# kocurvik/mdrp

Hardware: NVIDIA B200
Metric: image_pairs_per_sec (higher is better)
Workload: dtype f64

## Files before the change

mdrp_b200/csrc/repose_b200.cu:

```cuda
#include <cuda.h>
#include <cuda_runtime.h>
#include <algorithm>
#include <cstdio>
#include <cstdlib>
#include <cstring>
#include <string>
#include <type_traits>
#include <vector>

#include "rp_kernels.cuh"

using namespace rp;

namespace {

std::string g_create_error;

struct DevBuf {
    void *p = nullptr;
    size_t cap = 0;
    cudaError_t reserve(size_t bytes) {
        if (bytes <= cap) return cudaSuccess;
        if (p) cudaFree(p);
        p = nullptr;
// ... 3 lines not shown
        if (e == cudaSuccess) cap = want;
        return e;
    }
    void release() {
        if (p) cudaFree(p);
        p = nullptr;
        cap = 0;
    }
    template <class T>
    T *as() const { return (T *)p; }
};

enum { B_OFFS, B_PAIRS, B_PTS64, B_PTS32, B_BEAR, B_SAMPLES, B_MODELS, B_HYPITER, B_SCORE, B_COUNT, B_SEGCNT,
       B_ITEMPFX, B_SCALARS, B_EVENTS, B_NEVENTS, B_LOMODELS, B_LOOFEV, B_LOCOUNT, B_PROBLIST, B_LOSCORE,
       B_LOCNT, B_LOITEMPFX, B_BEST, B_FINSTART, B_FINSCORE, B_FINCNT, B_ONES, B_ONEPFX, B_ENABLE, B_STATS,
       B_PTS32P, B_UB, B_LB, B_FIRSTCNT, B_FIRSTPFX, B_B0, B_S0, B_SURVLIST, B_SURVCNT, B_SURVPFX, B_WAVECUR, B_WAVECNT,
       B_MASK, B_IN_X1, B_IN_X2, B_IN_D1, B_IN_D2, B_IN_CAMS, B_TMP0, B_TMP1, B_TMP2,
       B_MASK_B, B_IN_X1_B, B_IN_X2_B, B_IN_D1_B, B_IN_D2_B, B_IN_CAMS_B, B_TMP0_B, B_TMP1_B,
       B_FEAT, B_TCOUT, B_TCLIST, B_TCLISTCNT, B_TCLISTPFX, B_PAIRCNT, B_TCPFX, B_TCSPLIT,
       B_PAIRFLAGS, B_SUB_IDX, B_SUB_SRC, B_SUB_DST, B_SUB_X1, B_SUB_X2, B_SUB_D1, B_SUB_D2, B_SUB_CAMS, B_SUB_MODELS,
       B_SUB_STATS, B_SUB_MASK,
       B_STG_X1, B_STG_X2, B_STG_D1, B_STG_D2, B_STG_X1_B, B_STG_X2_B, B_STG_D1_B, B_STG_D2_B,
       B_QUAL, B_QUAL_B, B_ORDOFFS, B_ORDOFFS_B, B_PERM, B_PERM_B, B_KSORT, B_KSORT_B, B_ORDSCR,
       B_GATHER_Q, B_NBUF };

struct Scalars {
    int n_items, n_lo_items, n_one_items, n_prob, n_pairs_scalar, any_flag, reserved0, n_first_items;
    int n_surv_items, bound_work, lm_work, score_work;
    unsigned long long point_scores, lm_iters, n_survivors, evaluated_ps;
    long long n_hyp;
    int n_tc_items, n_tcsel_items;
    unsigned long long tc_evaluated, tc_selected, lm_flops;
};

constexpr int N_EVENTS = 29;

}

struct rp_ctx {
    int device = 0;
    int sms = 148;
    std::string err;
    int64_t launches = 0;
    cudaStream_t stream = nullptr;
    cudaStream_t copy_stream = nullptr;
    DevBuf buf[B_NBUF];
    cudaEvent_t ev[N_EVENTS];
    double last_ms[16] = {0};
    double prev_h2d_ms = 0.0, prev_dev_ms = 0.0;
    int64_t last_cnt[16] = {0};
    size_t workspace_budget = (size_t)80 << 30;
    bool prune = true;
    int head = HB;
    bool waves = true;
    int lm_warp = 0xf;
    int head_small = 32;
    int mid_end = 256;
    int mid_ends[4] = {256, 0, 0, 0}, n_mid = 1;
    bool tc = true;
    int tc_two_pass = -115;
    void *encode_tiled = nullptr;
    int ev_cap0 = EV;
    std::vector<int32_t> pair_status;
    int occ_score[4] = {0}, occ_lm[4] = {0};
};

namespace {

#define CK(call)                                                                                     \
    do {                                                                                             \
        cudaError_t e_ = (call);                                                                     \
        if (e_ != cudaSuccess) {                                                                     \
            char b_[512];                                                                            \
            snprintf(b_, sizeof b_, "%s failed at %s:%d: %s", #call, __FILE__, __LINE__,             \
                     cudaGetErrorString(e_));                                                        \
            ctx->err = b_;                                                                           \
            return RP_ERR_CUDA;                                                                      \
        }                                                                                            \
// ... 55 lines not shown
    }
    LAUNCHED();
    return RP_OK;
}

int launch_bound(rp_ctx *ctx, bool pose, const BoundArgs &a, cudaStream_t st) {
    CK(cudaMemsetAsync(a.work_counter, 0, sizeof(int), st));
    if (pose) bound_kernel<true><<<occupancy_grid(ctx, bound_kernel<true>, SCORE_THREADS), SCORE_THREADS, 0, st>>>(a);
    else bound_kernel<false><<<occupancy_grid(ctx, bound_kernel<false>, SCORE_THREADS), SCORE_THREADS, 0, st>>>(a);
    LAUNCHED();
    return RP_OK;
}

int launch_lm(rp_ctx *ctx, int variant, const LMArgs &a, long long expected_problems, cudaStream_t st) {
    ctx->launches++;
    (void)expected_problems;
    LMArgs la = a;
    la.work_counter = &ctx->buf[B_SCALARS].as<Scalars>()->lm_work;
    la.warp_kernel = (ctx->lm_warp >> variant) & 1;
    la.warp_single = (ctx->lm_warp >> 4) & 1;
    CK(cudaMemsetAsync(la.work_counter, 0, sizeof(int), st));
    CK((cudaError_t)launch_lm_kernel(ctx->sms, variant, la, st));
    return RP_OK;
}

int launch_solve(rp_ctx *ctx, int variant, const SolveArgs &a, int n_pairs, cudaStream_t st) {
    dim3 grid(a.nseg, n_pairs);
    const bool generic = getenv("RP_SOLVE_GENERIC") != nullptr;
    switch (variant) {
    case RP_CALIB:
        if (generic) solve_kernel<RP_CALIB><<<grid, SOLVE_THREADS, 0, st>>>(a);
        else solve2_kernel<P3PCand><<<grid, SOLVE_THREADS, 0, st>>>(a);
        break;
    case RP_CALIB_SHIFT:
        if (generic) solve_kernel<RP_CALIB_SHIFT><<<grid, SOLVE_THREADS, 0, st>>>(a);
        else solve2_kernel<ShiftCand><<<grid, SOLVE_THREADS, 0, st>>>(a);
        break;
    case RP_SHARED:
        if (generic) solve_kernel<RP_SHARED><<<grid, SOLVE_THREADS, 0, st>>>(a);
        else solve2_kernel<FocalCand><<<grid, SOLVE_THREADS, 0, st>>>(a);
        break;
    default: solve_kernel<RP_VARYING><<<grid, SOLVE_THREADS, 0, st>>>(a); break;
    }
    LAUNCHED();
    return RP_OK;
}
// ... 77 lines not shown
    CK(B[B_PAIRFLAGS].reserve(sizeof(int) * P));
    CK(B[B_LOCNT].reserve(sizeof(int) * (size_t)P * ev_cap));
    CK(B[B_LOITEMPFX].reserve(sizeof(int) * (P + 1)));
    CK(B[B_BEST].reserve(sizeof(Model) * P));
    CK(B[B_FINSTART].reserve(sizeof(Model) * P));
    CK(B[B_FINSCORE].reserve(sizeof(double) * P));
    CK(B[B_FINCNT].reserve(sizeof(int) * P));
    CK(B[B_ONES].reserve(sizeof(int) * P));
    CK(B[B_ONEPFX].reserve(sizeof(int) * (P + 1)));
    CK(B[B_ENABLE].reserve(sizeof(int) * P));
    CK(B[B_STATS].reserve(sizeof(rp_stats) * P));
    if (ctx->prune) {
        CK(B[B_UB].reserve(sizeof(int) * slots));
        CK(B[B_LB].reserve(sizeof(float) * slots));
        CK(B[B_SURVLIST].reserve(sizeof(int) * slots));
        CK(B[B_FIRSTCNT].reserve(sizeof(int) * P));
        CK(B[B_FIRSTPFX].reserve(sizeof(int) * (P + 1)));
        CK(B[B_B0].reserve(sizeof(int) * P));
        CK(B[B_S0].reserve(sizeof(double) * P));
        CK(B[B_SURVCNT].reserve(sizeof(int) * P));
        CK(B[B_WAVECUR].reserve(sizeof(int) * P)); CK(B[B_WAVECNT].reserve(sizeof(int) * P));
        CK(B[B_SURVPFX].reserve(sizeof(int) * (P + 1)));
    }
    const bool use_tc = ctx->prune && ctx->tc;
    if (use_tc) {
        CK(B[B_FEAT].reserve(128 * (size_t)std::max<long long>(N, 1) + 128 * tc::NT));
        CK(B[B_TCOUT].reserve(sizeof(int) * slots));
        CK(B[B_TCLIST].reserve(sizeof(int) * slots));
        CK(B[B_TCLISTCNT].reserve(sizeof(int) * P));
        CK(B[B_TCLISTPFX].reserve(sizeof(int) * (P + 1)));
        CK(B[B_PAIRCNT].reserve(sizeof(int) * P));
        CK(B[B_TCSPLIT].reserve(sizeof(int) * P));
        CK(B[B_TCPFX].reserve(sizeof(int) * (P + 1)));
    }

    Scalars *sc = B[B_SCALARS].as<Scalars>();
    PairParams *pairs = B[B_PAIRS].as<PairParams>();
    Pt64 *pts64 = B[B_PTS64].as<Pt64>();
    float4 *pts32 = B[B_PTS32].as<float4>();
    Bear *bear = B[B_BEAR].as<Bear>();
    int *samples = B[B_SAMPLES].as<int>();
    Model *models = B[B_MODELS].as<Model>();
    int *hyp_iter = B[B_HYPITER].as<int>();
    double *score = B[B_SCORE].as<double>();
    int *count = B[B_COUNT].as<int>();
    int *seg_count = B[B_SEGCNT].as<int>();
// ... 185 lines not shown
    {
        ScanArgs a;
        a.n_pairs = P; a.nseg = nseg; a.seg_count = seg_count; a.score = score; a.count = count;
        a.events = B[B_EVENTS].as<int>(); a.n_events = B[B_NEVENTS].as<int>(); a.ev_cap = ev_cap;
        a.pair_flags = B[B_PAIRFLAGS].as<int>(); a.any_flag = &sc->any_flag;
        scan_kernel<<<cdiv((long long)P * 32, 256), 256, 0, st>>>(a);
        LAUNCHED();
        LoPrepArgs l;
        l.n_pairs = P; l.nseg = nseg; l.events = a.events; l.n_events = a.n_events; l.hyp_iter = hyp_iter; l.ev_cap = ev_cap;
        l.models = models; l.lo_models = B[B_LOMODELS].as<Model>(); l.lo_of_event = B[B_LOOFEV].as<int>();
        l.lo_count = B[B_LOCOUNT].as<int>(); l.prob_list = B[B_PROBLIST].as<int>(); l.n_prob = &sc->n_prob;
        lo_prepare_kernel<<<cdiv(P, 128), 128, 0, st>>>(l);
        LAUNCHED();
    }
    CK(cudaEventRecord(ev[5], st));
    LMArgs la;
    memset(&la, 0, sizeof la);
    la.pairs = pairs; la.pts64 = pts64; la.d1 = io.d1; la.d2 = io.d2;
    la.weight_sampson = opt.weight_sampson; la.gradient_tol = 1e-10; la.step_tol = 1e-8;
    la.initial_lambda = 1e-3; la.min_lambda = 1e-10; la.max_lambda = 1e10;
    la.loss_scale_override = -1.0; la.scale_reproj_override = -1.0;
    la.lm_iters = &sc->lm_iters;
    la.lm_flops = &sc->lm_flops;
    {
        la.prob_list = B[B_PROBLIST].as<int>(); la.n_prob = &sc->n_prob; la.prob_per_pair = ev_cap;
        la.models = B[B_LOMODELS].as<Model>(); la.use_final = 0;
        int rc = launch_lm(ctx, variant, la, (long long)P * 8, st);
        if (rc) return rc;
    }
    CK(cudaEventRecord(ev[6], st));
    {
        build_items_kernel<<<1, 1024, 0, st>>>(P, B[B_LOCOUNT].as<int>(), B[B_LOITEMPFX].as<int>(), &sc->n_lo_items, nullptr);
        LAUNCHED();
        ScoreArgs s2 = sa;
        s2.slot_list = nullptr; s2.list_stride = 0;
        s2.n_groups = P; s2.grp_stride = ev_cap; s2.grp_per_pair = 1; s2.grp_cnt = B[B_LOCOUNT].as<int>();
        s2.item_prefix = B[B_LOITEMPFX].as<int>(); s2.n_items = &sc->n_lo_items; s2.models = B[B_LOMODELS].as<Model>();
        s2.score = B[B_LOSCORE].as<double>(); s2.count = B[B_LOCNT].as<int>(); s2.point_scores = nullptr;
        int rc = launch_score(ctx, pose, false, s2, st);
        if (rc) return rc;
        MergeArgs m;
        m.n_pairs = P; m.nseg = nseg; m.iters = iters; m.pairs = pairs; m.events = B[B_EVENTS].as<int>();
        m.min_iterations = opt.min_iterations; m.max_iterations = opt.max_iterations;
        m.dyn_num_trials_mult = opt.dyn_num_trials_mult; m.log_prob_missing = log(1.0 - opt.success_prob);
        m.hyp_iter = hyp_iter; m.ev_cap = ev_cap; m.pair_flags = B[B_PAIRFLAGS].as<int>(); m.any_flag = &sc->any_flag;
        m.n_events = B[B_NEVENTS].as<int>(); m.lo_of_event = B[B_LOOFEV].as<int>(); m.score = score; m.count = count;
// ... 143 lines not shown

int rerun_flagged(rp_ctx *ctx, int variant, const rp_options &opt, const ChunkIO &io, const std::vector<long long> &rel,
                  const std::vector<int> &flags0, int iters0, int64_t p0, cudaStream_t st) {
    DevBuf *B = ctx->buf;
    const bool pose = variant == RP_CALIB || variant == RP_CALIB_SHIFT;
    std::vector<int> todo;
    for (int i = 0; i < io.n_pairs; ++i)
        if (flags0[(size_t)i]) todo.push_back(i);
    int iters = iters0, ev_cap = ctx->ev_cap0;
    std::vector<int> flags_of((size_t)io.n_pairs, 0);
    for (int i : todo) flags_of[(size_t)i] = flags0[(size_t)i];
    while (!todo.empty()) {
        bool any_more = false, any_ovf = false;
        for (int i : todo) {
            any_more |= (flags_of[(size_t)i] & PAIR_FLAG_NEED_MORE) != 0;
            any_ovf |= (flags_of[(size_t)i] & PAIR_FLAG_OVERFLOW) != 0;
            ctx->pair_status[(size_t)(p0 + i)] |= ((flags_of[(size_t)i] & PAIR_FLAG_NEED_MORE) ? RP_PAIR_CONTINUED : 0) |
                                                  ((flags_of[(size_t)i] & PAIR_FLAG_OVERFLOW) ? RP_PAIR_EVENTS_RERUN : 0);
        }
        if (any_more) iters = (int)std::min<int64_t>(opt.max_iterations, (int64_t)iters * 4);
        const int slots_pp = std::max(1, cdiv(iters, SEG)) * 4 * SEG;
        if (any_ovf) ev_cap = (int)std::min<int64_t>((int64_t)ev_cap * 8, slots_pp);
        std::vector<int> next;
        size_t pos = 0;
        while (pos < todo.size()) {
            size_t end = pos;
            size_t bytes = 0;
            long long npts = 0;
            while (end < todo.size()) {
                const long long n = rel[(size_t)todo[end] + 1] - rel[(size_t)todo[end]];
                const size_t b = bytes_per_pair(iters, n, ev_cap);
                if (end > pos && bytes + b > ctx->workspace_budget) break;
                bytes += b;
                npts += n;
                ++end;
            }
            const int S = (int)(end - pos);
            std::vector<int> idx((size_t)S);
            std::vector<long long> src((size_t)S), dst((size_t)S + 1, 0);
            for (int j = 0; j < S; ++j) {
                idx[(size_t)j] = todo[pos + j];
                src[(size_t)j] = rel[(size_t)idx[(size_t)j]];
                dst[(size_t)j + 1] = dst[(size_t)j] + (rel[(size_t)idx[(size_t)j] + 1] - rel[(size_t)idx[(size_t)j]]);
            }
            const size_t nn = (size_t)std::max<long long>(npts, 1);
            int rc = RP_OK;
            std::vector<int> flags;
            do {
                cudaError_t e = cudaSuccess;
                (void)e;
// ... 56 lines not shown
                  cudaStream_t st) {
    constexpr bool f32 = std::is_same<In, float>::value;
    const bool ordered = quality != nullptr;
    const bool staged = f32 || ordered;
    int rc = check_common(ctx, variant, n_pairs, offsets, opt_in);
    if (rc) return rc;
    CK(cudaSetDevice(ctx->device));
    rp_options opt = *opt_in;
    if (variant == RP_CALIB && opt.estimate_shift) variant = RP_CALIB_SHIFT;
    if (variant == RP_CALIB_SHIFT) opt.estimate_shift = 1;
    const bool pose = variant == RP_CALIB || variant == RP_CALIB_SHIFT;
    if (pose && !cams && n_pairs > 0) return fail(ctx, RP_ERR_INVALID, "calibrated variants need cams");
    memset(ctx->last_ms, 0, sizeof ctx->last_ms);
    memset(ctx->last_cnt, 0, sizeof ctx->last_cnt);
    ctx->pair_status.assign((size_t)n_pairs, RP_PAIR_OK);
    if (n_pairs == 0) return RP_OK;
    const long long Ntot = offsets[n_pairs] - offsets[0];
    const int iters0 = opt.min_iterations < opt.max_iterations
                           ? (int)std::min<int64_t>(opt.max_iterations, opt.min_iterations + 1)
                           : (int)opt.max_iterations;
    size_t in_bytes = f32 ? 48 : 0;
    if (ordered) in_bytes = host_io ? 2 * (6 * sizeof(In) + 4 + 4 + 1) : 48 + 4 + 1;
    const size_t bpp = bytes_per_pair(iters0, Ntot / n_pairs + 1, ctx->ev_cap0, in_bytes);
    int64_t chunk = (int64_t)std::max<size_t>(1, ctx->workspace_budget / bpp);
    chunk = std::min<int64_t>(chunk, 32768);
    std::vector<long long> rel;
    DevBuf *B = ctx->buf;
    std::vector<int64_t> bounds(1, 0);
    {
        int64_t first = 0;
        if (host_io && n_pairs >= 1024 && !getenv("RP_NO_LEAD_CHUNK")) {
            double f = 0.125;
            if (ctx->prev_h2d_ms > 0.0 && ctx->prev_dev_ms > 0.0) f = ctx->prev_h2d_ms / (ctx->prev_h2d_ms + ctx->prev_dev_ms);
            f = std::min(1.0 / 3.0, std::max(1.0 / 32.0, f));
            first = std::min<int64_t>(std::min<int64_t>(n_pairs, chunk), std::max<int64_t>(256, (int64_t)(f * (double)n_pairs)));
        }
        if (first > 0) bounds.push_back(first);
        const int64_t rest = n_pairs - first;
        const int64_t k = (rest + chunk - 1) / chunk;
        for (int64_t i = 1; i <= k; ++i) bounds.push_back(first + (rest * i) / k);
    }
    const int64_t n_chunks = (int64_t)bounds.size() - 1;
    static const int IN_X1[2] = {B_IN_X1, B_IN_X1_B}, IN_X2[2] = {B_IN_X2, B_IN_X2_B}, IN_D1[2] = {B_IN_D1, B_IN_D1_B},
                     IN_D2[2] = {B_IN_D2, B_IN_D2_B}, IN_CAMS[2] = {B_IN_CAMS, B_IN_CAMS_B}, OUT_M[2] = {B_TMP0, B_TMP0_B},
                     OUT_S[2] = {B_TMP1, B_TMP1_B}, OUT_K[2] = {B_MASK, B_MASK_B};
    static const int STG_X1[2] = {B_STG_X1, B_STG_X1_B}, STG_X2[2] = {B_STG_X2, B_STG_X2_B}, STG_D1[2] = {B_STG_D1, B_STG_D1_B},
                     STG_D2[2] = {B_STG_D2, B_STG_D2_B};
// ... 188 lines not shown
    }
    if (device < 0 || device >= ndev) {
        g_create_error = "device index out of range";
        return RP_ERR_INVALID;
    }
    cudaDeviceProp prop;
    if (cudaGetDeviceProperties(&prop, device) != cudaSuccess || prop.major < 10) {
        g_create_error = "device is not sm_100-class (this library only ships sm_100a code)";
        return RP_ERR_NO_DEVICE;
    }
    rp_ctx *ctx = new rp_ctx();
    ctx->device = device;
    ctx->sms = prop.multiProcessorCount;
    if (cudaSetDevice(device) != cudaSuccess || cudaStreamCreateWithFlags(&ctx->stream, cudaStreamNonBlocking) != cudaSuccess ||
        cudaStreamCreateWithFlags(&ctx->copy_stream, cudaStreamNonBlocking) != cudaSuccess) {
        g_create_error = "cudaSetDevice / stream creation failed";
        delete ctx;
        return RP_ERR_CUDA;
    }
    for (auto &ev : ctx->ev) cudaEventCreate(&ev);
    if (const char *np = getenv("RP_NO_PRUNE")) ctx->prune = !(np[0] == '1');
    if (const char *nw = getenv("RP_NO_WAVES")) ctx->waves = !(nw[0] == '1');
    if (const char *lw = getenv("RP_LM_WARP")) ctx->lm_warp = atoi(lw) & 0x1f;
    if (const char *hs = getenv("RP_HEAD_SMALL")) { const int v = atoi(hs); if (v >= 0 && v <= 256 && v % 32 == 0) ctx->head_small = v; }
    if (const char *me = getenv("RP_MID_END")) {
        int n = 0, vals[4] = {0, 0, 0, 0};
        bool ok = true;
        for (const char *p = me; *p && n < 4;) {
            const int v = atoi(p);
            if (v < 0 || v > SEG || v % 32 != 0 || (n && v <= vals[n - 1])) ok = false;
            vals[n++] = v;
            while (*p && *p != ',') ++p;
            if (*p == ',') ++p;
        }
        if (ok && n) { ctx->n_mid = n; for (int k = 0; k < 4; ++k) ctx->mid_ends[k] = vals[k]; ctx->mid_end = vals[n - 1]; }
    }
    if (const char *nt = getenv("RP_NO_TC")) ctx->tc = !(nt[0] == '1');
    if (const char *sp = getenv("RP_TC_SPLIT")) { const int v = atoi(sp); if (v >= 1 && v <= 15) ctx->tc_two_pass = v; }
    if (const char *ap = getenv("RP_TC_ADAPT_PCT")) { const int v = atoi(ap); if (v >= 50 && v <= 200) ctx->tc_two_pass = -v; }
    if (const char *op = getenv("RP_TC_ONE_PASS")) { if (op[0] == '1') ctx->tc_two_pass = 0; }
    if (const char *ec = getenv("RP_EV_CAP")) { const int v = atoi(ec); if (v >= 1 && v <= EV) ctx->ev_cap0 = v; }
    {
        cudaDriverEntryPointQueryResult qres;
        void *fn = nullptr;
        if (cudaGetDriverEntryPoint("cuTensorMapEncodeTiled", &fn, cudaEnableDefault, &qres) != cudaSuccess || !fn ||
            qres != cudaDriverEntryPointSuccess ||
// ... 549 lines not shown
```

mdrp_b200/csrc/repose_lm.cu:

```cuda
#include "rp_lm_kernel.cuh"

#ifndef RP_LM_THREADS
#define RP_LM_THREADS 128
#endif

namespace rp {

template <class K>
static int occupancy_grid(int sms, K kernel, int threads) {
    int nb = 0;
    if (cudaOccupancyMaxActiveBlocksPerMultiprocessor(&nb, kernel, threads, 0) != cudaSuccess || nb < 1) nb = 1;
    return nb * sms;
}

template <int VARIANT, int NP>
static void launch_variant(int sms, const LMArgs &a, cudaStream_t st) {
    if (a.warp_kernel && (a.prob_list || a.warp_single) && !a.mask && !a.use_final)
        lm_warp_kernel<VARIANT, NP, RP_LOSS_TRUNCATED>
            <<<occupancy_grid(sms, lm_warp_kernel<VARIANT, NP, RP_LOSS_TRUNCATED>, LMW_WPB[VARIANT] * 32), LMW_WPB[VARIANT] * 32, 0, st>>>(a);
    else if (!a.use_final)
        lm_kernel<VARIANT, NP, RP_LM_THREADS, RP_LOSS_TRUNCATED>
            <<<occupancy_grid(sms, lm_kernel<VARIANT, NP, RP_LM_THREADS, RP_LOSS_TRUNCATED>, RP_LM_THREADS), RP_LM_THREADS, 0, st>>>(a);
    else if (a.loss_type == RP_LOSS_TRUNCATED_CAUCHY)
        lm_kernel<VARIANT, NP, RP_LM_THREADS, RP_LOSS_TRUNCATED_CAUCHY>
            <<<occupancy_grid(sms, lm_kernel<VARIANT, NP, RP_LM_THREADS, RP_LOSS_TRUNCATED_CAUCHY>, RP_LM_THREADS), RP_LM_THREADS, 0, st>>>(a);
    else if (a.loss_type == RP_LOSS_CAUCHY)
        lm_kernel<VARIANT, NP, RP_LM_THREADS, RP_LOSS_CAUCHY>
            <<<occupancy_grid(sms, lm_kernel<VARIANT, NP, RP_LM_THREADS, RP_LOSS_CAUCHY>, RP_LM_THREADS), RP_LM_THREADS, 0, st>>>(a);
    else
        lm_kernel<VARIANT, NP, RP_LM_THREADS, -1>
            <<<occupancy_grid(sms, lm_kernel<VARIANT, NP, RP_LM_THREADS, -1>, RP_LM_THREADS), RP_LM_THREADS, 0, st>>>(a);
}

int launch_lm_kernel(int sms, int variant, const LMArgs &a, cudaStream_t st) {
    switch (variant) {
    case RP_CALIB: launch_variant<RP_CALIB, 7>(sms, a, st); break;
    case RP_CALIB_SHIFT: launch_variant<RP_CALIB_SHIFT, 9>(sms, a, st); break;
    case RP_SHARED: launch_variant<RP_SHARED, 8>(sms, a, st); break;
    default: launch_variant<RP_VARYING, 9>(sms, a, st); break;
    }
    return (int)cudaGetLastError();
}

}
```

mdrp_b200/csrc/rp_lm.cuh:

```cuda
#pragma once
#include "rp_common.cuh"

namespace rp {

RP_HD double loss_eval(int type, double thr, double r2) {
    const double t2 = thr * thr;
    switch (type) {
    case RP_LOSS_TRIVIAL: return r2;
    case RP_LOSS_TRUNCATED: return t2 < r2 ? t2 : r2;
    case RP_LOSS_HUBER: { const double r = sqrt(r2); return r <= thr ? r2 : thr * (2.0 * r - thr); }
    case RP_LOSS_CAUCHY: return t2 * log1p(r2 / t2);
    case RP_LOSS_TRUNCATED_CAUCHY: return r2 > t2 ? t2 * log1p(1.0) : t2 * log1p(r2 / t2);
    default: return r2 < t2 ? r2 : t2;
    }
}
RP_HD double loss_weight(int type, double thr, double r2) {
    const double t2 = thr * thr;
    switch (type) {
    case RP_LOSS_TRIVIAL: return 1.0;
    case RP_LOSS_TRUNCATED: return r2 < t2 ? 1.0 : 0.0;
    case RP_LOSS_HUBER: { const double r = sqrt(r2); return r <= thr ? 1.0 : thr / r; }
    case RP_LOSS_CAUCHY: return 1.0 / (1.0 + r2 / t2);
    case RP_LOSS_TRUNCATED_CAUCHY: return r2 > t2 ? 0.0 : 1.0 / (1.0 + r2 / t2);
    default: return r2 < t2 ? 1.0 : 0.0;
// ... 148 lines not shown
                        fma_(R.r0.z, qx, fma_(R.r1.z, qy, R.r2.z)));
        const double a = d1 + F.shift1;
        const V3 Z = v3(fma_(a, s.x, F.t.x), fma_(a, s.y, F.t.y), fma_(a, s.z, F.t.z));
        if (Z.z > 0.0) {
            const double iz = lm_rcp(Z.z);
            const double r0 = f2 * (Z.x * iz) - x2_0, r1 = f2 * (Z.y * iz) - x2_1;
            cost += robust_cost<LOSS, false>(P, loss_type, P.scale_reproj * (r0 * r0 + r1 * r1), lp);
        }
        const double b = F.scale * (d2 + F.shift2);
        const V3 Y = v3(fma_(b, m.x, -F.Rt.x), fma_(b, m.y, -F.Rt.y), fma_(b, m.z, -F.Rt.z));
        if (Y.z > 0.0) {
            const double iz = lm_rcp(Y.z);
            const double r0 = f1 * (Y.x * iz) - x1_0, r1 = f1 * (Y.y * iz) - x1_1;
            cost += robust_cost<LOSS, false>(P, loss_type, P.scale_reproj * (r0 * r0 + r1 * r1), lp);
        }
    }
    return cost;
}

constexpr int LM_FLOPS[4][4] = {{104, 146, 131, 182}, {104, 146, 162, 222}, {112, 201, 183, 244}, {112, 220, 217, 286}};

template <int VARIANT, int NP, int LOSS = -1>
RP_HD double point_eval(const LMFrame &F, const LMParams &P, double x1_0, double x1_1, double x2_0,
                        double x2_1, double d1, double d2, NormalEq<NP> &N, unsigned long long &rows, LogProd &lp) {
    constexpr bool FOCAL = (VARIANT == RP_SHARED || VARIANT == RP_VARYING);
    const int loss_type = LOSS >= 0 ? LOSS : P.loss_type;
    const double f1 = FOCAL ? F.f1 : 1.0, f2 = FOCAL ? F.f2 : 1.0;
    const double if1sq = FOCAL ? F.if1sq : 1.0, if2sq = FOCAL ? F.if2sq : 1.0;
    constexpr int CF2 = (VARIANT == RP_SHARED) ? 7 : 8;
    constexpr unsigned M_POSE = 0x3Fu;
    constexpr unsigned M_FOC = VARIANT == RP_SHARED ? 0x80u : (VARIANT == RP_VARYING ? 0x180u : 0u);
    constexpr unsigned M_S = M_POSE | M_FOC;
    constexpr unsigned M_12 = M_POSE | M_FOC | (VARIANT == RP_CALIB_SHIFT ? 0x80u : 0u);
    constexpr unsigned M_21 = M_POSE | 0x40u | M_FOC | (VARIANT == RP_CALIB_SHIFT ? 0x100u : 0u);
    const double px = FOCAL ? x1_0 * F.if1 : x1_0, py = FOCAL ? x1_1 * F.if1 : x1_1;
    const double qx = FOCAL ? x2_0 * F.if2 : x2_0, qy = FOCAL ? x2_1 * F.if2 : x2_1;
    const M3 &R = F.R;
    const M3 &E = F.E;
    double J[NP];
    double cost = 0.0;
    const V3 s = v3(fma_(R.r0.x, px, fma_(R.r0.y, py, R.r0.z)), fma_(R.r1.x, px, fma_(R.r1.y, py, R.r1.z)),
                    fma_(R.r2.x, px, fma_(R.r2.y, py, R.r2.z)));
    const V3 m = v3(fma_(R.r0.x, qx, fma_(R.r1.x, qy, R.r2.x)), fma_(R.r0.y, qx, fma_(R.r1.y, qy, R.r2.y)),
                    fma_(R.r0.z, qx, fma_(R.r1.z, qy, R.r2.z)));

    if (P.weight_sampson > 0.0) {
        const V3 Ep1 = v3(fma_(E.r0.x, px, fma_(E.r0.y, py, E.r0.z)), fma_(E.r1.x, px, fma_(E.r1.y, py, E.r1.z)),
                          fma_(E.r2.x, px, fma_(E.r2.y, py, E.r2.z)));
        const V3 Etp2 = v3(fma_(E.r0.x, qx, fma_(E.r1.x, qy, E.r2.x)), fma_(E.r0.y, qx, fma_(E.r1.y, qy, E.r2.y)),
                           fma_(E.r0.z, qx, fma_(E.r1.z, qy, E.r2.z)));
        const double C = fma_(qx, Ep1.x, fma_(qy, Ep1.y, Ep1.z));
        const double A = Ep1.x * Ep1.x + Ep1.y * Ep1.y, B = Etp2.x * Etp2.x + Etp2.y * Etp2.y;
        const double inv = lm_rsqrt(A * if2sq + B * if1sq);
        const double rs = C * inv;
        cost += robust_cost<LOSS, true>(P, loss_type, rs * rs, lp);
        const double w = P.weight_sampson * P.weight_sampson *
                         robust_weight<LOSS>(P, loss_type, FOCAL ? P.weight_sampson * (rs * rs) : rs * rs);
        if (w != 0.0) {
#pragma unroll
            for (int i = 0; i < NP; ++i) J[i] = 0.0;
            const double c2 = rs * inv;
            const double a2 = if2sq, a1 = if1sq;
            {
// ... 19 lines not shown
            {
                const double tx = qx * R.r2.x - R.r0.x, ty = qx * R.r2.y - R.r0.y;
                const double dC = qx * s.z - s.x;
                J[4] = dC - c2 * ((Ep1.x * s.z) * a2 + (Etp2.x * tx + Etp2.y * ty) * a1);
            }
            {
                const double tx = qy * R.r0.x - qx * R.r1.x, ty = qy * R.r0.y - qx * R.r1.y;
                const double dC = qy * s.x - qx * s.y;
                J[5] = dC - c2 * ((Ep1.y * s.x - Ep1.x * s.y) * a2 + (Etp2.x * tx + Etp2.y * ty) * a1);
            }
            if (FOCAL) {
                const double dpx = -px * F.if1, dpy = -py * F.if1, dqx = -qx * F.if2, dqy = -qy * F.if2;
                const double e1x = E.r0.x * dpx + E.r0.y * dpy, e1y = E.r1.x * dpx + E.r1.y * dpy;
                const double e2x = E.r0.x * dqx + E.r1.x * dqy, e2y = E.r0.y * dqx + E.r1.y * dqy;
                const double j1 = (Etp2.x * dpx + Etp2.y * dpy) -
                                  c2 * ((Ep1.x * e1x + Ep1.y * e1y) * a2 - B * a1 * F.if1);
                const double j2 = (Ep1.x * dqx + Ep1.y * dqy) -
                                  c2 * ((Etp2.x * e2x + Etp2.y * e2y) * a1 - A * a2 * F.if2);
                if (VARIANT == RP_SHARED) J[7] = j1 + j2;
                else { J[7] = j1; J[CF2] = j2; }
            }
            N.template add_row<M_S>(w * (inv * inv), J, C);
            rows += 1ull;
        }
    }
    if (!(P.scale_reproj > 0.0)) return cost;

    {
        const double a = d1 + F.shift1;
        const V3 Z = v3(fma_(a, s.x, F.t.x), fma_(a, s.y, F.t.y), fma_(a, s.z, F.t.z));
        if (Z.z > 0.0) {
            const double iz = lm_rcp(Z.z);
            const double u0 = Z.x * iz, u1 = Z.y * iz;
            const double r0 = f2 * u0 - x2_0, r1 = f2 * u1 - x2_1;
            cost += robust_cost<LOSS, false>(P, loss_type, P.scale_reproj * (r0 * r0 + r1 * r1), lp);
            const double w = P.scale_reproj * robust_weight<LOSS>(P, loss_type, P.scale_reproj * (r0 * r0 + r1 * r1));
            if (w != 0.0) {
                const double g = f2 * iz;
                const double zg = FOCAL ? Z.z * F.if2 : Z.z;
                double J0[NP], J1[NP];
#pragma unroll
                for (int i = 0; i < NP; ++i) { J0[i] = 0.0; J1[i] = 0.0; }
                {
                    const double dx = py * R.r0.z - R.r0.y, dy = py * R.r1.z - R.r1.y, dz = py * R.r2.z - R.r2.y;
                    J0[0] = a * (dx - u0 * dz); J1[0] = a * (dy - u1 * dz);
                }
                {
                    const double dx = R.r0.x - px * R.r0.z, dy = R.r1.x - px * R.r1.z, dz = R.r2.x - px * R.r2.z;
                    J0[1] = a * (dx - u0 * dz); J1[1] = a * (dy - u1 * dz);
                }
                {
                    const double dx = px * R.r0.y - py * R.r0.x, dy = px * R.r1.y - py * R.r1.x, dz = px * R.r2.y - py * R.r2.x;
                    J0[2] = a * (dx - u0 * dz); J1[2] = a * (dy - u1 * dz);
                }
                J0[3] = 1.0; J0[5] = -u0;
                J1[4] = 1.0; J1[5] = -u1;
                if (VARIANT == RP_CALIB_SHIFT) {
                    J0[7] = s.x - u0 * s.z; J1[7] = s.y - u1 * s.z;
                }
                if (FOCAL) {
                    const double ex = -(a * px) * F.if1, ey = -(a * py) * F.if1;
                    const double dx = R.r0.x * ex + R.r0.y * ey, dy = R.r1.x * ex + R.r1.y * ey, dz = R.r2.x * ex + R.r2.y * ey;
                    J0[7] = dx - u0 * dz; J1[7] = dy - u1 * dz;
                    J0[CF2] += Z.x * F.if2; J1[CF2] += Z.y * F.if2;
                }
                const double sw = w * (g * g);
                N.template add_row<(M_12 & ~0x10u)>(sw, J0, r0 * zg);
                N.template add_row<(M_12 & ~0x08u)>(sw, J1, r1 * zg);
                rows += 1ull << 21;
            }
        }
    }
    {
        const double bb = d2 + F.shift2;
        const double b = F.scale * bb;
        const V3 Y = v3(fma_(b, m.x, -F.Rt.x), fma_(b, m.y, -F.Rt.y), fma_(b, m.z, -F.Rt.z));
        if (Y.z > 0.0) {
            const double iz = lm_rcp(Y.z);
            const double u0 = Y.x * iz, u1 = Y.y * iz;
            const double r0 = f1 * u0 - x1_0, r1 = f1 * u1 - x1_1;
            cost += robust_cost<LOSS, false>(P, loss_type, P.scale_reproj * (r0 * r0 + r1 * r1), lp);
            const double w = P.scale_reproj * robust_weight<LOSS>(P, loss_type, P.scale_reproj * (r0 * r0 + r1 * r1));
            if (w != 0.0) {
                const double g = f1 * iz;
                const double zg = FOCAL ? Y.z * F.if1 : Y.z;
                double J0[NP], J1[NP];
#pragma unroll
                for (int i = 0; i < NP; ++i) { J0[i] = 0.0; J1[i] = 0.0; }
                J0[0] = u0 * Y.y;            J1[0] = Y.z + u1 * Y.y;
                J0[1] = -Y.z - u0 * Y.x;     J1[1] = -u1 * Y.x;
                J0[2] = Y.y;                 J1[2] = -Y.x;
                J0[3] = u0 * R.r0.z - R.r0.x; J1[3] = u1 * R.r0.z - R.r0.y;
                J0[4] = u0 * R.r1.z - R.r1.x; J1[4] = u1 * R.r1.z - R.r1.y;
                J0[5] = u0 * R.r2.z - R.r2.x; J1[5] = u1 * R.r2.z - R.r2.y;
                const double m0 = m.x - u0 * m.z, m1 = m.y - u1 * m.z;
                J0[6] = bb * m0; J1[6] = bb * m1;
                if (VARIANT == RP_CALIB_SHIFT) { J0[8] = F.scale * m0; J1[8] = F.scale * m1; }
                if (FOCAL) {
                    const double ex = -b * qx * F.if2, ey = -b * qy * F.if2;
                    const double dx = R.r0.x * ex + R.r1.x * ey, dy = R.r0.y * ex + R.r1.y * ey, dz = R.r0.z * ex + R.r1.z * ey;
                    J0[CF2] += dx - u0 * dz; J1[CF2] += dy - u1 * dz;
                    J0[7] += Y.x * F.if1; J1[7] += Y.y * F.if1;
                }
                const double sw = w * (g * g);
                N.template add_row<M_21>(sw, J0, r0 * zg);
                N.template add_row<M_21>(sw, J1, r1 * zg);
                rows += 1ull << 42;
            }
        }
    }
    return cost;
}

template <int VARIANT, int NP>
RP_HD void point_accumulate(const LMFrame &F, const LMParams &P, double x1_0, double x1_1, double x2_0,
                            double x2_1, double d1, double d2, NormalEq<NP> &N) {
    unsigned long long rows = 0;
    LogProd lp;
    lp.init();
    (void)point_eval<VARIANT, NP>(F, P, x1_0, x1_1, x2_0, x2_1, d1, d2, N, rows, lp);
}

template <int VARIANT>
RP_HD Model model_step(const Model &m, const double *dp) {
    Model o = m;
    o.q = quat_mul(m.q, quat_exp(v3(dp[0], dp[1], dp[2])));
    o.t = v3(m.t.x + dp[3], m.t.y + dp[4], m.t.z + dp[5]);
    o.scale = m.scale + dp[6];
    if (VARIANT == RP_CALIB_SHIFT) { o.shift1 = m.shift1 + dp[7]; o.shift2 = m.shift2 + dp[8]; }
    if (VARIANT == RP_SHARED) { o.f1 = m.f1 + dp[7]; o.f2 = o.f1; }
    if (VARIANT == RP_VARYING) { o.f1 = m.f1 + dp[7]; o.f2 = m.f2 + dp[8]; }
    return o;
}

template <int NP>
RP_HD void llt_solve(const double *A, double lambda, const double *b, double *x) {
    double L[NP * (NP + 1) / 2], inv[NP];
#pragma unroll
    for (int j = 0; j < NP; ++j) {
        double s = A[j * (j + 1) / 2 + j] + lambda;
#pragma unroll
        for (int k = 0; k < j; ++k) s -= L[j * (j + 1) / 2 + k] * L[j * (j + 1) / 2 + k];
        const double d = sqrt(s);
// ... 29 lines not shown
```

mdrp_b200/csrc/rp_lm_kernel.cuh:

```cuda
#pragma once
#include "rp_types.cuh"
#include "rp_lm.cuh"
#include <type_traits>

#ifndef RP_LM_UNROLL
#define RP_LM_UNROLL 1
#endif
#ifndef RP_LM_MIN_BLOCKS
#define RP_LM_MIN_BLOCKS 3
#endif

namespace rp {

constexpr int LM_UNROLL = RP_LM_UNROLL;

struct LMArgs {
    const int *prob_list;
    const int *n_prob;
    int prob_per_pair;
    const PairParams *pairs;
    const Pt64 *pts64;
    const double *d1, *d2;
    const unsigned char *mask;
    const int *enable;
    Model *models;
    int use_final;
    int max_iterations, loss_type;
    double weight_sampson, gradient_tol, step_tol, initial_lambda, min_lambda, max_lambda;
    double loss_scale_override;
    double scale_reproj_override;
    rp_bundle_stats *stats;
    unsigned long long *lm_iters;
    unsigned long long *lm_flops;
    int *work_counter;
    int warp_kernel;
    int warp_single;
};

constexpr int LM_LIST_CAP = 16384;

template <int MAXV, int CNT, int O>
struct ReduceScatter {
    static RP_D void run(double (&v)[MAXV], int lane, int &base, int &lim) {
        constexpr int H = (CNT + 1) / 2;
        const bool up = (lane & O) != 0;
#pragma unroll
        for (int i = 0; i < H; ++i) {
            const double lo = v[i];
            const double hi = (i + H < CNT) ? v[i + H] : 0.0;
            const double send = up ? lo : hi, keep = up ? hi : lo;
            v[i] = keep + __shfl_xor_sync(0xffffffffu, send, O);
        }
        if (up) { base += H; lim = max(lim - H, 0); }
        else lim = min(lim, H);
        ReduceScatter<MAXV, H, O / 2>::run(v, lane, base, lim);
    }
};
template <int MAXV, int CNT>
struct ReduceScatter<MAXV, CNT, 0> {
// ... 94 lines not shown
            }
            if (lm_loss_may_be_cauchy(LOSS)) c += P.loss_scale * P.loss_scale * lp.total(P.weight_sampson);
            c = warp_sum(c);
            __syncthreads();
            if (lane == 0) cred[wid] = c;
            __syncthreads();
            double tot = 0.0;
#pragma unroll
            for (int w = 0; w < LM_WARPS; ++w) tot += cred[w];
            return tot;
        };

        auto block_eval = [&](const Model &m, NormalEq<NP> &N) -> double {
            const LMFrame F = make_frame(m);
            double c = 0.0;
            LogProd lp;
            lp.init();
            N.clear();
#pragma unroll LM_UNROLL
            for (int i = tid; i < m_work; i += LM_THREADS) {
                const int k = use_list ? (int)list_s[i] : i;
                if (!use_list && mask && !mask[k]) continue;
                const Pt64 p = pts[k];
                c += point_eval<VARIANT, NP, LOSS>(F, P, p.x1_0, p.x1_1, p.x2_0, p.x2_1, d1[k], d2[k], N, rows, lp);
            }
            if (lm_loss_may_be_cauchy(LOSS)) c += P.loss_scale * P.loss_scale * lp.total(P.weight_sampson);
            c = warp_sum(c);
            __syncthreads();
            if (lane == 0) cred[wid] = c;
            __syncthreads();
            double tot = 0.0;
#pragma unroll
            for (int w = 0; w < LM_WARPS; ++w) tot += cred[w];
            return tot;
        };
        auto reduce_normal = [&](NormalEq<NP> &N) {
            constexpr int NV = NA + NP, LEFT = ReduceScatterLeft<NV, 5>::value;
            double v[NV];
#pragma unroll
            for (int i = 0; i < NA; ++i) v[i] = N.A[i];
#pragma unroll
            for (int i = 0; i < NP; ++i) v[NA + i] = N.g[i];
            int base = 0, lim = NV;
            ReduceScatter<NV, NV, 16>::run(v, lane, base, lim);
            __syncthreads();
#pragma unroll
            for (int j = 0; j < LEFT; ++j)
// ... 124 lines not shown
        if (lane == 0) pj = atomicAdd(a.work_counter, 1);
        pj = __shfl_sync(0xffffffffu, pj, 0);
        if (pj >= n_prob) break;
        const int prob = a.prob_list ? a.prob_list[pj] : pj;
        const int pair = prob / a.prob_per_pair;
        const PairParams pp = a.pairs[pair];
        if (!pp.valid) continue;
        if (a.enable && !a.enable[pair]) continue;
        LMParams P;
        P.weight_sampson = a.weight_sampson;
        P.scale_reproj = a.scale_reproj_override >= 0.0 ? a.scale_reproj_override : pp.scale_reproj;
        if (a.use_final) {
            P.loss_type = LOSS >= 0 ? LOSS : a.loss_type;
            P.loss_scale = a.loss_scale_override > 0.0 ? a.loss_scale_override : pp.final_loss_scale;
        } else {
            P.loss_type = RP_LOSS_TRUNCATED;
            P.loss_scale = pp.lo_loss_scale;
        }
        P.inv_t2 = 1.0 / (P.loss_scale * P.loss_scale);
        const int max_it = a.use_final ? a.max_iterations : 25;
        const int n = pp.n;
        const Pt64 *pts = a.pts64 + pp.off;
        const double *d1 = a.d1 + pp.off, *d2 = a.d2 + pp.off;
        __syncwarp();
        if (lane == 0) { W.cur = a.models[prob]; W.stop = 0; }
        __syncwarp();

        auto fetch = [&](int i, int s) {
            if (i < n) {
                Slot *d = &ring[s][lane];
                const char *src = reinterpret_cast<const char *>(pts + i);
                cp_async16(&d->x[0], src);
                cp_async16(&d->x[2], src + 16);
                cp_async8(&d->d1, d1 + i);
                cp_async8(&d->d2, d2 + i);
            }
            cp_async_commit();
        };

        unsigned long long rows = 0;
        auto warp_pass = [&](const Model &m, NormalEq<NP> &N, auto jac_tag) -> double {
            constexpr bool jac = decltype(jac_tag)::value;
            const LMFrame F = make_frame(m);
            double c = 0.0;
            LogProd lp;
            lp.init();
            if (jac) N.clear();
            fetch(lane, 0);
            fetch(lane + 32, 1);
            int s = 0;
            for (int i = lane; i < n; i += 32) {
                cp_async_wait<1>();
                const Slot q = ring[s][lane];
                int s2 = s + 2; if (s2 >= LMW_SLOTS) s2 -= LMW_SLOTS;
                fetch(i + 64, s2);
                if (jac) c += point_eval<VARIANT, NP, LOSS>(F, P, q.x[0], q.x[1], q.x[2], q.x[3], q.d1, q.d2, N, rows, lp);
                else c += point_cost<VARIANT, LOSS>(F, P, q.x[0], q.x[1], q.x[2], q.x[3], q.d1, q.d2, lp);
                if (++s == LMW_SLOTS) s = 0;
            }
            cp_async_wait<0>();
            if (lm_loss_may_be_cauchy(LOSS)) c += P.loss_scale * P.loss_scale * lp.total(P.weight_sampson);
            return warp_sum(c);
        };
        auto reduce_normal = [&](NormalEq<NP> &N) {
            constexpr int NV = NA + NP, LEFT = ReduceScatterLeft<NV, 5>::value;
            double v[NV];
#pragma unroll
            for (int i = 0; i < NA; ++i) v[i] = N.A[i];
#pragma unroll
            for (int i = 0; i < NP; ++i) v[NA + i] = N.g[i];
            int base = 0, lim = NV;
            ReduceScatter<NV, NV, 16>::run(v, lane, base, lim);
            __syncwarp();
#pragma unroll
            for (int j = 0; j < LEFT; ++j)
                if (j < lim) { const int e = base + j; if (e < NA) W.sA[e] = v[j]; else W.sg[e - NA] = v[j]; }
            __syncwarp();
        };

        NormalEq<NP> N;
        int passes = 0;
        double cost;
        if (max_it > 0) { cost = warp_pass(W.cur, N, std::true_type{}); reduce_normal(N); }
        else cost = warp_pass(W.cur, N, std::false_type{});
        ++passes;
        const double initial_cost = cost;
        double lambda = a.initial_lambda;
        double grad_norm = -1.0, step_norm = -1.0;
        long long invalid_steps = 0;
        bool recompute = true;
        int it = 0;
        for (; it < max_it; ++it) {
            if (recompute) {
                double g2 = 0.0;
#pragma unroll
                for (int i = 0; i < NP; ++i) g2 += W.sg[i] * W.sg[i];
                grad_norm = sqrt(g2);
                if (grad_norm < a.gradient_tol) break;
            }
            if (lane == 0) {
                double x[NP];
                llt_solve<NP>(W.sA, lambda, W.sg, x);
                double sn = 0.0;
#pragma unroll
                for (int i = 0; i < NP; ++i) { x[i] = -x[i]; sn += x[i] * x[i]; }
                W.step_norm = sqrt(sn);
                if (sqrt(sn) < a.step_tol) W.stop = 1;
                else W.trial = model_step<VARIANT>(W.cur, x);
            }
            __syncwarp();
            step_norm = W.step_norm;
            if (W.stop) break;
            const bool last = it == max_it - 1;
            const double cost_new = last ? warp_pass(W.trial, N, std::false_type{}) : warp_pass(W.trial, N, std::true_type{});
            ++passes;
            if (cost_new < cost) {
                __syncwarp();
                if (lane == 0) W.cur = W.trial;
                lambda = fmax(a.min_lambda, lambda / 10);
                cost = cost_new;
                if (!last) reduce_normal(N);
                recompute = true;
            } else {
                ++invalid_steps;
                lambda = fmin(a.max_lambda, lambda * 10);
                recompute = false;
            }
            __syncwarp();
        }
        __syncwarp();
        if (lane == 0) {
            a.models[prob] = W.cur;
            if (a.stats) {
                rp_bundle_stats s;
                s.iterations = it; s.initial_cost = initial_cost; s.cost = cost; s.lambda = lambda;
                s.invalid_steps = invalid_steps; s.step_norm = step_norm; s.grad_norm = grad_norm;
                a.stats[prob] = s;
            }
            if (a.lm_iters) atomicAdd(a.lm_iters, (unsigned long long)it);
        }
        if (a.lm_flops) {
#pragma unroll
            for (int o = 16; o > 0; o >>= 1) rows += __shfl_xor_sync(0xffffffffu, rows, o);
            if (lane == 0) {
                const unsigned long long fl = (rows & 0x1fffffull) * LM_FLOPS[VARIANT][1] + ((rows >> 21) & 0x1fffffull) * LM_FLOPS[VARIANT][2] +
                                              ((rows >> 42) & 0x1fffffull) * LM_FLOPS[VARIANT][3] +
                                              (unsigned long long)passes * n * LM_FLOPS[VARIANT][0];
                atomicAdd(a.lm_flops, fl);
            }
        }
    }
}

int launch_lm_kernel(int sms, int variant, const LMArgs &a, cudaStream_t st);

}
```

Measured before the change: 80320.

## Reorder LM warp points by residual class to reduce divergence

Each Jacobian pass of the warp-level LM kernel now records a per-point class bitmask saying which residual blocks were active. Before the next Jacobian pass, the warp builds a stable counting-sort permutation that groups points of the same class, and the pass then visits points in that order. The aim is to cut warp divergence in point_eval across the Sampson and reprojection branches. In exchange it adds a per-warp scratch buffer sized from occupancy, an order-building sweep each iteration, indirect gathers, and workspace budget that is subtracted from chunk sizing.

```diff
diff --git a/mdrp_b200/csrc/repose_b200.cu b/mdrp_b200/csrc/repose_b200.cu
--- a/mdrp_b200/csrc/repose_b200.cu
+++ b/mdrp_b200/csrc/repose_b200.cu
@@ -49,7 +49,8 @@
        B_SUB_STATS, B_SUB_MASK,
        B_STG_X1, B_STG_X2, B_STG_D1, B_STG_D2, B_STG_X1_B, B_STG_X2_B, B_STG_D1_B, B_STG_D2_B,
        B_QUAL, B_QUAL_B, B_ORDOFFS, B_ORDOFFS_B, B_PERM, B_PERM_B, B_KSORT, B_KSORT_B, B_ORDSCR,
-       B_GATHER_Q, B_NBUF };
+       B_GATHER_Q,
+       B_LMORDER, B_NBUF };
 
 struct Scalars {
     int n_items, n_lo_items, n_one_items, n_prob, n_pairs_scalar, any_flag, reserved0, n_first_items;
@@ -81,6 +82,7 @@
     int head = HB;
     bool waves = true;
     int lm_warp = 0xf;
+    bool lm_order = true;
     int head_small = 32;
     int mid_end = 256;
     int mid_ends[4] = {256, 0, 0, 0}, n_mid = 1;
@@ -182,6 +184,14 @@
     CK(cudaMemsetAsync(la.work_counter, 0, sizeof(int), st));
     CK((cudaError_t)launch_lm_kernel(ctx->sms, variant, la, st));
     return RP_OK;
+}
+
+size_t lm_order_stride(rp_ctx *ctx, int variant, long long max_n) {
+    if (!ctx->lm_order || !((ctx->lm_warp >> variant) & 1)) return 0;
+    return (size_t)(std::min<long long>(max_n, LM_ORDER_CAP) + 3) / 4 * 4;
+}
+size_t lm_order_bytes(rp_ctx *ctx, int variant, long long max_n) {
+    return 5 * lm_order_stride(ctx, variant, max_n) * (size_t)lm_warp_slots(ctx->sms, variant);
 }
 
 int launch_solve(rp_ctx *ctx, int variant, const SolveArgs &a, int n_pairs, cudaStream_t st) {
@@ -305,6 +315,10 @@
         CK(B[B_WAVECUR].reserve(sizeof(int) * P)); CK(B[B_WAVECNT].reserve(sizeof(int) * P));
         CK(B[B_SURVPFX].reserve(sizeof(int) * (P + 1)));
     }
+    long long max_n = 0;
+    for (int p = 0; p < P; ++p) max_n = std::max(max_n, io.h_offsets_rel[p + 1] - io.h_offsets_rel[p]);
+    const int lm_stride = (int)lm_order_stride(ctx, variant, max_n);
+    if (lm_stride > 0) CK(B[B_LMORDER].reserve(lm_order_bytes(ctx, variant, max_n)));
     const bool use_tc = ctx->prune && ctx->tc;
     if (use_tc) {
         CK(B[B_FEAT].reserve(128 * (size_t)std::max<long long>(N, 1) + 128 * tc::NT));
@@ -536,6 +550,10 @@
     la.loss_scale_override = -1.0; la.scale_reproj_override = -1.0;
     la.lm_iters = &sc->lm_iters;
     la.lm_flops = &sc->lm_flops;
+    if (lm_stride > 0) {
+        la.order = B[B_LMORDER].as<int>();
+        la.order_stride = lm_stride;
+    }
     {
         la.prob_list = B[B_PROBLIST].as<int>(); la.n_prob = &sc->n_prob; la.prob_per_pair = ev_cap;
         la.models = B[B_LOMODELS].as<Model>(); la.use_final = 0;
@@ -725,10 +743,13 @@
         const int slots_pp = std::max(1, cdiv(iters, SEG)) * 4 * SEG;
         if (any_ovf) ev_cap = (int)std::min<int64_t>((int64_t)ev_cap * 8, slots_pp);
         std::vector<int> next;
+        long long max_n = 0;
+        for (int i : todo) max_n = std::max(max_n, rel[(size_t)i + 1] - rel[(size_t)i]);
+        const size_t lm_fixed = lm_order_bytes(ctx, variant, max_n);
         size_t pos = 0;
         while (pos < todo.size()) {
             size_t end = pos;
-            size_t bytes = 0;
+            size_t bytes = lm_fixed;
             long long npts = 0;
             while (end < todo.size()) {
                 const long long n = rel[(size_t)todo[end] + 1] - rel[(size_t)todo[end]];
@@ -831,7 +852,10 @@
     size_t in_bytes = f32 ? 48 : 0;
     if (ordered) in_bytes = host_io ? 2 * (6 * sizeof(In) + 4 + 4 + 1) : 48 + 4 + 1;
     const size_t bpp = bytes_per_pair(iters0, Ntot / n_pairs + 1, ctx->ev_cap0, in_bytes);
-    int64_t chunk = (int64_t)std::max<size_t>(1, ctx->workspace_budget / bpp);
+    long long max_n = 0;
+    for (int64_t p = 0; p < n_pairs; ++p) max_n = std::max<long long>(max_n, offsets[p + 1] - offsets[p]);
+    const size_t lm_fixed = std::min(lm_order_bytes(ctx, variant, max_n), ctx->workspace_budget / 2);
+    int64_t chunk = (int64_t)std::max<size_t>(1, (ctx->workspace_budget - lm_fixed) / bpp);
     chunk = std::min<int64_t>(chunk, 32768);
     std::vector<long long> rel;
     DevBuf *B = ctx->buf;
@@ -1066,6 +1090,7 @@
     if (const char *np = getenv("RP_NO_PRUNE")) ctx->prune = !(np[0] == '1');
     if (const char *nw = getenv("RP_NO_WAVES")) ctx->waves = !(nw[0] == '1');
     if (const char *lw = getenv("RP_LM_WARP")) ctx->lm_warp = atoi(lw) & 0x1f;
+    if (const char *lo = getenv("RP_LM_ORDER")) ctx->lm_order = !(lo[0] == '0');
     if (const char *hs = getenv("RP_HEAD_SMALL")) { const int v = atoi(hs); if (v >= 0 && v <= 256 && v % 32 == 0) ctx->head_small = v; }
     if (const char *me = getenv("RP_MID_END")) {
         int n = 0, vals[4] = {0, 0, 0, 0};
diff --git a/mdrp_b200/csrc/repose_lm.cu b/mdrp_b200/csrc/repose_lm.cu
--- a/mdrp_b200/csrc/repose_lm.cu
+++ b/mdrp_b200/csrc/repose_lm.cu
@@ -32,6 +32,20 @@
             <<<occupancy_grid(sms, lm_kernel<VARIANT, NP, RP_LM_THREADS, -1>, RP_LM_THREADS), RP_LM_THREADS, 0, st>>>(a);
 }
 
+template <int VARIANT, int NP>
+static int warp_slots(int sms) {
+    return occupancy_grid(sms, lm_warp_kernel<VARIANT, NP, RP_LOSS_TRUNCATED>, LMW_WPB[VARIANT] * 32) * LMW_WPB[VARIANT];
+}
+
+int lm_warp_slots(int sms, int variant) {
+    switch (variant) {
+    case RP_CALIB: return warp_slots<RP_CALIB, 7>(sms);
+    case RP_CALIB_SHIFT: return warp_slots<RP_CALIB_SHIFT, 9>(sms);
+    case RP_SHARED: return warp_slots<RP_SHARED, 8>(sms);
+    default: return warp_slots<RP_VARYING, 9>(sms);
+    }
+}
+
 int launch_lm_kernel(int sms, int variant, const LMArgs &a, cudaStream_t st) {
     switch (variant) {
     case RP_CALIB: launch_variant<RP_CALIB, 7>(sms, a, st); break;
diff --git a/mdrp_b200/csrc/rp_lm.cuh b/mdrp_b200/csrc/rp_lm.cuh
--- a/mdrp_b200/csrc/rp_lm.cuh
+++ b/mdrp_b200/csrc/rp_lm.cuh
@@ -194,7 +194,8 @@
 
 template <int VARIANT, int NP, int LOSS = -1>
 RP_HD double point_eval(const LMFrame &F, const LMParams &P, double x1_0, double x1_1, double x2_0,
-                        double x2_1, double d1, double d2, NormalEq<NP> &N, unsigned long long &rows, LogProd &lp) {
+                        double x2_1, double d1, double d2, NormalEq<NP> &N, unsigned long long &rows, LogProd &lp,
+                        int &cls) {
     constexpr bool FOCAL = (VARIANT == RP_SHARED || VARIANT == RP_VARYING);
     const int loss_type = LOSS >= 0 ? LOSS : P.loss_type;
     const double f1 = FOCAL ? F.f1 : 1.0, f2 = FOCAL ? F.f2 : 1.0;
@@ -211,6 +212,7 @@
     const M3 &E = F.E;
     double J[NP];
     double cost = 0.0;
+    cls = 0;
     const V3 s = v3(fma_(R.r0.x, px, fma_(R.r0.y, py, R.r0.z)), fma_(R.r1.x, px, fma_(R.r1.y, py, R.r1.z)),
                     fma_(R.r2.x, px, fma_(R.r2.y, py, R.r2.z)));
     const V3 m = v3(fma_(R.r0.x, qx, fma_(R.r1.x, qy, R.r2.x)), fma_(R.r0.y, qx, fma_(R.r1.y, qy, R.r2.y)),
@@ -276,6 +278,7 @@
             }
             N.template add_row<M_S>(w * (inv * inv), J, C);
             rows += 1ull;
+            cls |= 1;
         }
     }
     if (!(P.scale_reproj > 0.0)) return cost;
@@ -322,6 +325,7 @@
                 N.template add_row<(M_12 & ~0x10u)>(sw, J0, r0 * zg);
                 N.template add_row<(M_12 & ~0x08u)>(sw, J1, r1 * zg);
                 rows += 1ull << 21;
+                cls |= 2;
             }
         }
     }
@@ -360,6 +364,7 @@
                 N.template add_row<M_21>(sw, J0, r0 * zg);
                 N.template add_row<M_21>(sw, J1, r1 * zg);
                 rows += 1ull << 42;
+                cls |= 4;
             }
         }
     }
@@ -372,7 +377,8 @@
     unsigned long long rows = 0;
     LogProd lp;
     lp.init();
-    (void)point_eval<VARIANT, NP>(F, P, x1_0, x1_1, x2_0, x2_1, d1, d2, N, rows, lp);
+    int cls;
+    (void)point_eval<VARIANT, NP>(F, P, x1_0, x1_1, x2_0, x2_1, d1, d2, N, rows, lp, cls);
 }
 
 template <int VARIANT>
diff --git a/mdrp_b200/csrc/rp_lm_kernel.cuh b/mdrp_b200/csrc/rp_lm_kernel.cuh
--- a/mdrp_b200/csrc/rp_lm_kernel.cuh
+++ b/mdrp_b200/csrc/rp_lm_kernel.cuh
@@ -35,6 +35,8 @@
     int *work_counter;
     int warp_kernel;
     int warp_single;
+    int *order;
+    int order_stride;
 };
 
 constexpr int LM_LIST_CAP = 16384;
@@ -175,7 +177,8 @@
                 const int k = use_list ? (int)list_s[i] : i;
                 if (!use_list && mask && !mask[k]) continue;
                 const Pt64 p = pts[k];
-                c += point_eval<VARIANT, NP, LOSS>(F, P, p.x1_0, p.x1_1, p.x2_0, p.x2_1, d1[k], d2[k], N, rows, lp);
+                int cls;
+                c += point_eval<VARIANT, NP, LOSS>(F, P, p.x1_0, p.x1_1, p.x2_0, p.x2_1, d1[k], d2[k], N, rows, lp, cls);
             }
             if (lm_loss_may_be_cauchy(LOSS)) c += P.loss_scale * P.loss_scale * lp.total(P.weight_sampson);
             c = warp_sum(c);
@@ -346,43 +349,97 @@
         const int n = pp.n;
         const Pt64 *pts = a.pts64 + pp.off;
         const double *d1 = a.d1 + pp.off, *d2 = a.d2 + pp.off;
+        int *const order = a.order && n <= a.order_stride
+                               ? a.order + (size_t)(blockIdx.x * LMW_WPB[VARIANT] + wid) * (size_t)(a.order_stride + a.order_stride / 4)
+                               : nullptr;
+        auto cls = [&]() { return reinterpret_cast<unsigned char *>(order + a.order_stride); };
         __syncwarp();
         if (lane == 0) { W.cur = a.models[prob]; W.stop = 0; }
         __syncwarp();
 
-        auto fetch = [&](int i, int s) {
-            if (i < n) {
+        auto fetch = [&](int k, int s) {
+            if (k < n) {
                 Slot *d = &ring[s][lane];
-                const char *src = reinterpret_cast<const char *>(pts + i);
+                const char *src = reinterpret_cast<const char *>(pts + k);
                 cp_async16(&d->x[0], src);
                 cp_async16(&d->x[2], src + 16);
-                cp_async8(&d->d1, d1 + i);
-                cp_async8(&d->d2, d2 + i);
+                cp_async8(&d->d1, d1 + k);
+                cp_async8(&d->d2, d2 + k);
             }
             cp_async_commit();
         };
+        auto build_order = [&]() {
+            const unsigned lt = (1u << lane) - 1u;
+            const unsigned *cw = reinterpret_cast<const unsigned *>(cls());
+            int cursor = 0;
+            for (int sweep = 0; sweep < 2; ++sweep) {
+                for (int blk = 0; blk < n; blk += 256) {
+                    unsigned w[2];
+#pragma unroll
+                    for (int j = 0; j < 2; ++j) w[j] = blk + 128 * j + 4 * lane < n ? cw[blk / 4 + 32 * j + lane] : 0u;
+#pragma unroll
+                    for (int g = 0; g < 8; ++g) {
+                        const int b0 = blk + 32 * g;
+                        if (b0 >= n) break;
+                        const int k = b0 + lane;
+                        const bool valid = k < n;
+                        const unsigned v = __shfl_sync(0xffffffffu, w[g / 4], 8 * (g % 4) + (lane >> 2));
+                        const int c = valid ? (int)((v >> (8 * (lane & 3))) & 7u) : 0;
+                        const unsigned vm = __ballot_sync(0xffffffffu, valid);
+                        const unsigned m0 = __ballot_sync(0xffffffffu, c & 1), m1 = __ballot_sync(0xffffffffu, c & 2),
+                                       m2 = __ballot_sync(0xffffffffu, c & 4);
+                        auto of_class = [&](int q) { return vm & (q & 1 ? m0 : ~m0) & (q & 2 ? m1 : ~m1) & (q & 4 ? m2 : ~m2); };
+                        if (sweep == 1) {
+                            const int base = __shfl_sync(0xffffffffu, cursor, c);
+                            if (valid) order[base + __popc(of_class(c) & lt)] = k;
+                        }
+                        cursor += __popc(of_class(lane));
+                    }
+                }
+                if (sweep == 0) {
+                    int start = 0;
+#pragma unroll
+                    for (int q = 7; q > 0; --q) {
+                        const int cq = __shfl_sync(0xffffffffu, cursor, q);
+                        if (lane < q) start += cq;
+                    }
+                    cursor = start;
+                }
+            }
+            __syncwarp();
+        };
 
         unsigned long long rows = 0;
-        auto warp_pass = [&](const Model &m, NormalEq<NP> &N, auto jac_tag) -> double {
+        auto warp_pass = [&](const Model &m, NormalEq<NP> &N, auto jac_tag, bool ord) -> double {
             constexpr bool jac = decltype(jac_tag)::value;
             const LMFrame F = make_frame(m);
             double c = 0.0;
             LogProd lp;
             lp.init();
             if (jac) N.clear();
-            fetch(lane, 0);
-            fetch(lane + 32, 1);
+            auto index = [&](int i) { return ord && i < n ? order[i] : i; };
+            fetch(index(lane), 0);
+            fetch(index(lane + 32), 1);
+            int k_next = index(lane + 64);
             int s = 0;
             for (int i = lane; i < n; i += 32) {
+                const int k = ord ? order[i] : i;
                 cp_async_wait<1>();
                 const Slot q = ring[s][lane];
                 int s2 = s + 2; if (s2 >= LMW_SLOTS) s2 -= LMW_SLOTS;
-                fetch(i + 64, s2);
-                if (jac) c += point_eval<VARIANT, NP, LOSS>(F, P, q.x[0], q.x[1], q.x[2], q.x[3], q.d1, q.d2, N, rows, lp);
-                else c += point_cost<VARIANT, LOSS>(F, P, q.x[0], q.x[1], q.x[2], q.x[3], q.d1, q.d2, lp);
+                fetch(k_next, s2);
+                k_next = index(i + 96);
+                if (jac) {
+                    int cl;
+                    c += point_eval<VARIANT, NP, LOSS>(F, P, q.x[0], q.x[1], q.x[2], q.x[3], q.d1, q.d2, N, rows, lp, cl);
+                    if (order) cls()[k] = (unsigned char)cl;
+                } else {
+                    c += point_cost<VARIANT, LOSS>(F, P, q.x[0], q.x[1], q.x[2], q.x[3], q.d1, q.d2, lp);
+                }
                 if (++s == LMW_SLOTS) s = 0;
             }
             cp_async_wait<0>();
+            if (jac && order) __syncwarp();
             if (lm_loss_may_be_cauchy(LOSS)) c += P.loss_scale * P.loss_scale * lp.total(P.weight_sampson);
             return warp_sum(c);
         };
@@ -405,8 +462,8 @@
         NormalEq<NP> N;
         int passes = 0;
         double cost;
-        if (max_it > 0) { cost = warp_pass(W.cur, N, std::true_type{}); reduce_normal(N); }
-        else cost = warp_pass(W.cur, N, std::false_type{});
+        if (max_it > 0) { cost = warp_pass(W.cur, N, std::true_type{}, false); reduce_normal(N); }
+        else cost = warp_pass(W.cur, N, std::false_type{}, false);
         ++passes;
         const double initial_cost = cost;
         double lambda = a.initial_lambda;
@@ -436,7 +493,12 @@
             step_norm = W.step_norm;
             if (W.stop) break;
             const bool last = it == max_it - 1;
-            const double cost_new = last ? warp_pass(W.trial, N, std::false_type{}) : warp_pass(W.trial, N, std::true_type{});
+            double cost_new;
+            if (last) cost_new = warp_pass(W.trial, N, std::false_type{}, false);
+            else {
+                if (order) build_order();
+                cost_new = warp_pass(W.trial, N, std::true_type{}, order != nullptr);
+            }
             ++passes;
             if (cost_new < cost) {
                 __syncwarp();
@@ -477,5 +539,7 @@
 }
 
 int launch_lm_kernel(int sms, int variant, const LMArgs &a, cudaStream_t st);
+int lm_warp_slots(int sms, int variant);
+constexpr int LM_ORDER_CAP = 65536;
 
 }
```

After: 76320, median of 6. -5.0%, worse.
